# MeteoSwiss/flexpart

Hardware: AMD Instinct MI355X
Metric: particle-steps/sec (whole node) + achieved HBM GB/s, 1e8 particles (higher is better)
Workload: dtype f64

## Files before the change

__graft_entry__.py:

```python
from __future__ import annotations

import os
import subprocess
import sys

ROOT = os.path.dirname(os.path.abspath(__file__))
CSRC = os.path.join(ROOT, "flexpart_amd", "csrc")
HIPCC = os.environ.get("HIPCC", "/opt/rocm/bin/hipcc")


def _stale(out, srcs):
    if not os.path.exists(out):
        return True
    t = os.path.getmtime(out)
    return any(os.path.getmtime(s) > t for s in srcs)


UNITS = [(rb, part) for rb in (8, 4) for part in (0, 1, 2)]
HIPFLAGS = ["--offload-arch=gfx950", "-O3", "-std=c++17", "-fPIC",
            "-mllvm", "-disable-machine-licm"]


def build_library(force=False, only=None, extra_flags=(), tag=None):
    if extra_flags and not tag:
        raise ValueError("a build with extra flags needs a tag (it must not replace the product library)")
    srcs = [os.path.join(CSRC, f) for f in ("fpx_engine.hip", "fpx_device.hpp", "fpx_rng_host.hpp", "fpx_verttransform.hpp",
                                            "fpx_calcpar.hpp", "fpx_getvdep.hpp", "fpx_calcpv.hpp", "fpx_convect.hpp", "fpx_tu.hpp")]
    srcs.append(os.path.join(ROOT, "include", "flexpart_amd.h"))
    out = os.path.join(CSRC, f"libflexpart_amd_{tag}.so" if tag else "libflexpart_amd.so")
    objdir = os.path.join(CSRC, "build", tag) if tag else os.path.join(CSRC, "build")
    os.makedirs(objdir, exist_ok=True)
    flagrec = " ".join(HIPFLAGS + list(extra_flags))

    def stamp_ok(obj):
        try:
            return open(obj + ".flags").read() == flagrec
        except OSError:
            return False

    todo = []
    for rb, part in UNITS:
        name = f"r{rb}p{part}"
        obj = os.path.join(objdir, f"fpx_{name}.o")
        if only is not None and name not in only and os.path.exists(obj) and stamp_ok(obj):
            continue
        if only is not None and name in only or force or _stale(obj, srcs) or not stamp_ok(obj):
            todo.append((name, obj, rb, part))
    procs = []
    for name, obj, rb, part in todo:
        cmd = [HIPCC] + HIPFLAGS + list(extra_flags) + [f"-DFPX_TU_REAL={rb}", f"-DFPX_TU_PART={part}", "-c", os.path.join(CSRC, "fpx_engine.hip"), "-o", obj]
# ... 66 lines not shown
```

flexpart_amd/csrc/fpx_device.hpp:

```cpp
#pragma once
#include "fpx_tu.hpp"
#include <hip/hip_runtime.h>
#include <stdint.h>

namespace fpx {
FPX_TU_OPEN

#define K(x) ((R)(x))
#define FPX_DEV __device__ __forceinline__
#define FPX_HD __host__ __device__ __forceinline__

constexpr int kMaxSpec = 5;
constexpr int kMaxNests = 4;
constexpr int kDead = -999999999;

FPX_HD float m_exp(float x) { return expf(x); }
FPX_HD double m_exp(double x) { return exp(x); }
FPX_HD float m_log(float x) { return logf(x); }
FPX_HD double m_log(double x) { return log(x); }
FPX_HD float m_sqrt(float x) { return sqrtf(x); }
FPX_HD double m_sqrt(double x) { return sqrt(x); }
FPX_HD float m_fma(float a, float b, float c) { return fmaf(a, b, c); }
FPX_HD double m_fma(double a, double b, double c) { return fma(a, b, c); }
FPX_HD float m_sin(float x) { return sinf(x); }
FPX_HD double m_sin(double x) { return sin(x); }
FPX_HD float m_cos(float x) { return cosf(x); }
// ... 142 lines not shown
  const double f = fma(m, ic, -1.0);
  double p = m_fma_k(f, -1.0 / 6.0, 0.2);
  p = m_fma_k(f, p, -0.25);
  p = m_fma_k(f, p, 1.0 / 3.0);
  p = fma(f, p, -0.5);
  p = fma(f, p, 1.0);
  return fma((double)e, 6.93147180559945309417e-01, lc) + f * p;
}
FPX_DEV double m_log_abs(double x) { return m_log_abs(x, &kLogTab[0][0]); }
template <typename TP>
FPX_DEV double m_exp_tab(double x, TP tab ) {
  const double k = rint(x * 46.16624130844683);
  double r = fma(k, -0.02166084938653512, x);
  r = fma(k, -5.9631716539705866e-12, r);
  const int ki = (int)k;
  const double t = tab[ki & 31];
  double p = m_fma_k(r, 1.3888888888888888889e-03, 8.3333333333333333333e-03);
  p = m_fma_k(r, p, 4.1666666666666666667e-02);
  p = m_fma_k(r, p, 1.6666666666666666667e-01);
  p = fma(r, p, 0.5);
  p = fma(r, p, 1.0);
  return ldexp(fma(t, r * p, t), ki >> 5);
}
FPX_DEV double m_rcbrt(double x) {
  double r = (double)__builtin_amdgcn_exp2f(__log2f((float)x) * (-1.0f / 3.0f));
  const double third = 1.0 / 3.0;
#pragma unroll
  for (int it = 0; it < 2; it++) {
    const double e = fma(-(x * (r * r)), r, 1.0);
    r = fma(r * third, e, r);
  }
  return r;
}
FPX_DEV float m_expp(float x) { return __expf(x); }
FPX_DEV double m_expp(double x) {
  const double k = rint(x * 1.4426950408889634074);
  double r = fma(k, -6.93147180369123816490e-01, x);
  r = fma(k, -1.90821492927058770002e-10, r);
  const double r2 = r * r;
  double pe = fma(r2, 1.1470745597729724714e-11, 2.0876756987868098979e-09);
  pe = fma(r2, pe, 2.7557319223985890653e-07);
  pe = fma(r2, pe, 2.4801587301587301587e-05);
  pe = fma(r2, pe, 1.3888888888888888889e-03);
  pe = fma(r2, pe, 4.1666666666666666667e-02);
  pe = fma(r2, pe, 0.5);
  double po = fma(r2, 1.6059043836821614599e-10, 2.5052108385441718775e-08);
// ... 13 lines not shown
template <typename T>
FPX_DEV T m_erf_e(T x, T E) {
  const T ax = m_abs(x);
  const T xc = m_min(ax, (T)6.5);
  const T t = (xc - (T)3.0) * m_rcp(xc + (T)3.0);
  T p = (T)kErfC[0];
#pragma unroll
  for (int i = 1; i < 18; i++) p = p * t + (T)kErfC[i];
  const T r = (T)1.0 - E * p;
  return m_sign(r, x);
}
template <typename T>
FPX_DEV void m_erf_e2(T xa, T Ea, T xb, T Eb, T &ra, T &rb) {
  typedef const double __attribute__((address_space(4))) *const_ptr;
  const_ptr c = (const_ptr)kErfC;
  asm volatile("" : "+s"(c));
  const T aa = m_abs(xa), ab = m_abs(xb);
  const T ca = m_min(aa, (T)6.5), cb = m_min(ab, (T)6.5);
  const T ta = (ca - (T)3.0) * m_rcp(ca + (T)3.0), tb = (cb - (T)3.0) * m_rcp(cb + (T)3.0);
  T pa = (T)c[0], pb = (T)c[0];
#pragma unroll
  for (int i = 1; i < 18; i++) { const T k = (T)c[i]; pa = pa * ta + k; pb = pb * tb + k; }
  const T qa = (T)1.0 - Ea * pa, qb = (T)1.0 - Eb * pb;
  ra = m_sign(qa, xa);
  rb = m_sign(qb, xb);
}
FPX_DEV float m_powr(float x, float y) { return x > 0.0f ? expf(y * logf(x)) : powf(x, y); }
FPX_DEV double m_powr(double x, double y) { return m_expp(y * m_logp(x)); }
FPX_DEV float m_coslat(float x) { return cosf(x); }
FPX_DEV double m_coslat(double x) {
  if (!(fabs(x) < 1.7)) return cos(x);
  const double z = x * x;
  double p = -1.0 / 403291461126605635584000000.0;
  p = fma(p, z, 1.0 / 620448401733239439360000.0);
  p = fma(p, z, -1.0 / 1124000727777607680000.0);
  p = fma(p, z, 1.0 / 2432902008176640000.0);
  p = fma(p, z, -1.0 / 6402373705728000.0);
  p = fma(p, z, 1.0 / 20922789888000.0);
  p = fma(p, z, -1.0 / 87178291200.0);
  p = fma(p, z, 1.0 / 479001600.0);
  p = fma(p, z, -1.0 / 3628800.0);
  p = fma(p, z, 1.0 / 40320.0);
  p = fma(p, z, -1.0 / 720.0);
  p = fma(p, z, 1.0 / 24.0);
  p = fma(p, z, -0.5);
  return fma(p, z, 1.0);
// ... 592 lines not shown
  S_UST, S_WST2, S_OL, S_TRANS,
  S_IAUX, S_SIGU, S_ITLU,
  S_RHOAUX,
  S_NPASS,
  S_COUNT_LEAN,
  S_TDEP = S_COUNT_LEAN,
  S_SETCELL,
  S_SET_NUM, S_SET_DQ6, S_SET_V0,
  S_COUNT_AERO64,
  S_RT_TAG = S_COUNT_AERO64, S_RT_RHO1, S_RT_TT1, S_RT_RHO2, S_RT_TT2,
  S_COUNT
};
template <typename R> constexpr int stash_slots(bool lean, bool susp = true) { return lean ? (susp ? (int)S_COUNT_LEAN : (int)S_NPASS) : (sizeof(R) == 8 ? (int)S_COUNT_AERO64 : (int)S_COUNT); }
constexpr int kStashStride = 256;
template <typename R>
struct Stash {
  typedef __attribute__((address_space(3))) volatile R *lds_ptr;
  lds_ptr p;
  lds_tab_ptr tab;
  FPX_DEV double logabs(double x) const { return m_log_abs(x, tab); }
  FPX_DEV double expt(double x) const { return m_exp_tab(x, tab + kLdsExpTabAt); }
  FPX_DEV float logabs(float x) const { return m_logp(x); }
  FPX_DEV float expt(float x) const { return m_expp(x); }
  FPX_DEV R get(int k) const { return p[k * kStashStride]; }
  FPX_DEV void put(int k, R v) const { p[k * kStashStride] = v; }
  FPX_DEV void add(int k, R v) const { p[k * kStashStride] = p[k * kStashStride] + v; }
};

template <typename R>
FPX_DEV R inv_pack_itlu(const StepInv<R> &I) { return m_flip(I.itlu, (I.flags & INV_DEEP) ? 0x80000000u : 0u); }
FPX_DEV bool m_signbit(double x) { return __double2hiint(x) < 0; }
FPX_DEV bool m_signbit(float x) { return (int)__float_as_uint(x) < 0; }
template <typename R>
struct StashInv {
  const Stash<R> &S;
  FPX_DEV int regime() const { const R iaux = S.get(S_IAUX); return iaux > K(0.) ? 0 : iaux < K(0.) ? 1 : 2; }
  FPX_DEV bool deep() const { return m_signbit(S.get(S_ITLU)); }
  FPX_DEV R get_iaux() const { return S.get(S_IAUX); }
  FPX_DEV R get_sigu() const { return S.get(S_SIGU); }
  FPX_DEV R get_itlu() const { return m_abs(S.get(S_ITLU)); }
  FPX_DEV R get_wst2() const { return S.get(S_WST2); }
};

template <typename R>
struct HsInv {
  R ih, iaux;
  int regime;
};

template <typename R, typename ST>
// ... 29 lines not shown
    T.isigw = m_rcp(T.sigw);
    T.tlw = K(0.1) * T.h * T.isigw * m_pow08(T.zeta);
  }
  T.tlu = m_max(K(10.), T.tlu);
  T.tlv = m_max(K(10.), T.tlv);
  T.tlw = m_max(K(30.), T.tlw);
  if (sizeof(R) == 8) { if (__builtin_expect(T.dsigwdz == K(0.), 0)) { asm volatile("" ::: "memory"); T.dsigwdz = K(1.e-10); } }
  else if (T.dsigwdz == K(0.)) T.dsigwdz = K(1.e-10);
}

#define FPX_PI_PAR K(3.14159265)

template <typename R>
FPX_DEV R cuberoot(R x) { return m_sign(m_pow(m_abs(x), K(0.333333333)), x); }

template <typename R>
FPX_DEV R cbl_transition(R h, R ol) {
  R transition = K(1.);
  if (-h / ol < K(15)) transition = m_sin(((-h / ol + K(10.)) / K(10.)) * FPX_PI_PAR) / K(2.) + K(0.5);
  return transition;
}

template <typename R, typename ST>
FPX_DEV void cbl(const ST &S, int ldirect, R wp, R zp, R wt , R ih , R rhoaux , R sigmaw, R irw , R dsigmawdz, R tlw,
                 R &ath, R &bth, int &flagrein) {
  const R usurad2 = K(0.7071067812), usurad2p = K(0.3989422804), C0 = K(3), costluar4 = K(0.66667), eps = K(0.000001);
  const unsigned int tdir = ldirect < 0 ? 0x80000000u : 0u;
  const R z = zp * ih;
  const R w2 = sigmaw * sigmaw;
  const R rtl = m_rsqrt(tlw);
  const R alfa = (K(2.) / C0) * w2 * (rtl * rtl);
  const R wold = m_flip(wp, tdir);
  const R omz = K(1.) - z;
  const R omz05 = m_sqrtp(omz), omz15 = omz * omz05;
  const R w3 = (K(1.2) * z * omz15 + eps) * wt;
  const R dw3 = (K(1.2) * (omz15 - z * K(1.5) * omz05)) * (wt * ih);
  const R irw2 = irw * irw, irw3 = irw2 * irw;
  const R skew = w3 * irw3;
  const R dskew = irw3 * dw3 - K(3.) * skew * dsigmawdz * irw;
  R fluarw = K(0.), dfluarw = K(0.), xluarw = K(0.), dxluarw = K(0.);
  if (skew != K(0)) {
    R croot, icroot2;
    m_cuberoot_parts(m_abs(skew), croot, icroot2);
    fluarw = costluar4 * m_sign(croot, skew);
    dfluarw = costluar4 * (K(1.) / K(3.)) * icroot2 * dskew;
  }
  const R fluarw2 = fluarw * fluarw;
  const R a1 = K(1.) + fluarw2, a3 = K(3.) + fluarw2;
  const R ffd = K(2.) * fluarw * dfluarw;
  R a105, ia105;
  m_sqrt_rsqrt(a1, a105, ia105);
  if (skew != K(0)) {
    const R a115 = a1 * a105;
    const R ix = m_rcp(a3 * fluarw);
// ... 5 lines not shown
  m_sqrt_rsqrt(r4, r405, ir405);
  const R aluarw = K(0.5) * (K(1.) - xluarw * ir405);
  const R bluarw = K(1.) - aluarw;
  const R ir4 = ir405 * ir405;
  const R daluarw = K(-2.) * dxluarw * (ir405 * ir4);
  const R dbluarw = -daluarw;
  const R rs = r405 * ia105, rs3 = rs * (rs * rs);
  const R qa05 = bluarw * rs, qb05 = aluarw * rs;
  const R sigmawa = sigmaw * qa05, sigmawb = sigmaw * qb05;
  const R iv = irw * (a105 * r405);
  const R isa = iv * aluarw, isb = iv * bluarw;
  const R da1 = daluarw * a1, abf = ir4 * ffd, hs3 = K(0.5) * sigmaw * rs3;
  const R dsigmawa = dsigmawdz * qa05 - hs3 * bluarw * (da1 + abf);
  const R dsigmawb = dsigmawdz * qb05 + hs3 * aluarw * (da1 - abf);
  const R wa = fluarw * sigmawa, wb = fluarw * sigmawb;
  const R dwa = dfluarw * sigmawa + fluarw * dsigmawa;
  const R dwb = dfluarw * sigmawb + fluarw * dsigmawb;
  const R deltawa = wold - wa, deltawb = wold + wb;
  const R wold2 = wold * wold;
  const R isa2 = isa * isa, isb2 = isb * isb;
  const R da = deltawa * isa, db = deltawb * isb;
  if (m_abs(da) > K(6.) && m_abs(db) > K(6.)) flagrein = 1;
  const R da2 = da * da, db2 = db * db;
  const R ea = S.expt(-(K(0.5) * da2)), eb = S.expt(-(K(0.5) * db2));
  const R pa = (usurad2p * isa) * ea;
  const R pb = (usurad2p * isb) * eb;
  const R aperfa = da * usurad2;
  const R aperfb = db * usurad2;
  const R rx = rhoaux;
  const R apa = aluarw * pa, bpb = bluarw * pb;
  const R ptot = apa + bpb;
  const R Ta = aluarw * (dwa + wa * rx) + wa * daluarw;
  const R Tb = bluarw * (dwb + wb * rx) + wb * dbluarw;
  const R wdf = wold * dfluarw;
  const R Ua = sigmawa * (aluarw * (dsigmawa * (wold2 * isa2 + K(1.)) + wdf) + sigmawa * (daluarw + rx * aluarw));
  const R Ub = sigmawb * (bluarw * (dsigmawb * (wold2 * isb2 + K(1.)) - wdf) + sigmawb * (dbluarw + rx * bluarw));
  const R cu = usurad2 * usurad2 - K(0.5);
  R erfa, erfb;
  m_erf_e2(aperfa, ea - ea * (da2 * cu), aperfb, eb - eb * (db2 * cu), erfa, erfb);
  const R Phi = K(0.5) * (Tb * erfb - Ta * erfa) + Ua * pa + Ub * pb;
  const R Q = m_flip((da * isa) * apa + (db * isb) * bpb, tdir);
  ath = m_rcp(ptot) * (-(C0 / K(2.)) * alfa * Q + Phi);
  bth = (sigmaw * K(1.4142135623730951)) * rtl;
}

template <typename R>
FPX_DEV void cbl_pdf(R zp, R wst, R h, R sigmaw, R ol, R &aluarw, R &sigmawa, R &sigmawb, R &wa, R &wb) {
  const R costluar4 = K(0.66667), eps = K(0.000001);
  R z = zp / h;
  R transition = cbl_transition(h, ol);
  R w2 = sigmaw * sigmaw;
  const R omz = K(1.) - z;
  R w3 = ((K(1.2) * z * (omz * m_sqrt(omz)) + eps) * (wst * wst * wst)) * transition;
  R radw2 = m_sqrt(w2);
  R skew = w3 / (w2 * radw2);
  R skew2 = skew * skew;
  R fluarw = costluar4 * m_powr(skew, K(0.333333333333333));
  R fluarw2 = fluarw * fluarw;
  const R a1 = K(1.) + fluarw2, a3 = K(3.) + fluarw2;
  R rluarw = (a1 * a1 * a1) * skew2 / ((a3 * a3) * fluarw2);
  R xluarw = m_sqrt(rluarw);
  aluarw = K(0.5) * (K(1.) - xluarw / m_sqrt(K(4.) + rluarw));
  R bluarw = K(1.) - aluarw;
  sigmawa = radw2 * m_sqrt(bluarw / (aluarw * a1));
  sigmawb = radw2 * m_sqrt(aluarw / (bluarw * a1));
// ... 851 lines not shown
      const R y2 = k < 3 ? (h2 ? a3[lev][1][k] : a3[lev][0][k]) : (h2 ? a2[lev][1][k - 3] : a2[lev][0][k - 3]);
      y[k] = (y1 * W.dt2 + y2 * W.dt1) * W.dtt;
    }
#pragma unroll
    for (int k = 0; k < 5; k++) lv[lev][k] = y[k];
  }
}

constexpr int kRecStride = 16, kRecWst = 9;
template <typename R>
struct RecCold {
  const R *v0;
  unsigned int slot;
  FPX_DEV R wst() const {
    unsigned int s = slot;
    asm volatile("" : "+v"(s));
    return v0[(size_t)s * kRecStride + kRecWst];
  }
};

template <int T>
FPX_DEV bool sw(int runtime) { return T < 0 ? runtime != 0 : T != 0; }

template <typename R, bool DRYDEP, bool SETTLE, int TSW, int CBLF, typename RNG>
FPX_DEV int pbl_pass(const View<R> &V, const R *hgt, const RNG &G, const TimeW<R> &W, int itime, double xt, double yt,
                     R &zt, R &wp, int &ldt, short &icbt, LoopCtx<R> &A, const Stash<R> &S,
                     int &indz_last, Stats *st, const RecCold<R> &RC) {
  const R eps = V.eps;
  const R eps2 = K(1.e-9);
  const R href = K(15.);
  const R h = A.h;
  const Fld<R> F = fld_of(V, A.ngrid);
  int nrand = A.nrand;
  const bool turbswitch = sw<TSW>(V.turbswitch);
  const bool cblflag = sw<CBLF>(V.cblflag == 1);
  const bool turboff = TSW < 0 && V.turboff != 0;
  Turb<R> T;
  T.h = h;
  T.sigw = K(0.); T.dsigw2dz = K(0.); T.dsigwdz = K(0.);

  if (V.method == 1) {
    ldt = min(ldt, abs(V.lsynctime - A.itimec + itime));
    A.itimec = A.itimec + ldt * V.ldirect;
  } else {
    ldt = abs(V.lsynctime);
    A.itimec = itime + V.lsynctime;
  }
  const R dt = (R)ldt;
  T.zeta = zt / h;
// ... 48 lines not shown
    R au, bu, av, bv;
    factors(dt * itlu, au, bu);
    if (regime_h == 1) { av = au; bv = bu; }
    else factors(dt * itlv, av, bv);
    R up = S.get(S_UP), vp = S.get(S_VP);
    up = au * up + g1 * T.sigu * bu;
    vp = av * vp + g2 * T.sigv * bv;
    if (turboff) { up = K(0.); vp = K(0.); }
    S.put(S_UP, up); S.put(S_VP, vp);
    S.add(S_DAW, up * dt);
    S.add(S_DCW, vp * dt);
  }
  nrand = nrand + 2;

  if (nrand + V.ifine > V.maxrand) nrand = 1;
  const R dtf = dt * V.fine;
  const R dtftlw = dtf * m_rcp(T.tlw);
  const bool cbl_on = cblflag && SI.deep();
  const R sqrt_dtf = m_sqrtp(dtf);
  const HsInv<R> HI{ih, SI.get_iaux(), SI.regime()};

  FPX_LANES(st, 0);
  unsigned int flip = icbt < 0 ? 0x80000000u : 0u;
  for (int i = 1; i <= V.ifine; i++) {
    R delz;
    FPX_LANES(st, 1);
    if (turbswitch) {
      if (dtftlw < K(.5)) {
        if (cblflag) {
          if (cbl_on) {
            FPX_LANES(st, 2);
            int flagrein = 0;
            nrand = nrand + 1;
            R old_wp_buf = wp, ath, bth;
            cbl(S, V.ldirect, wp, zt, S.get(S_TRANS), HI.ih, S.get(S_RHOAUX), T.sigw, T.isigw, T.dsigwdz, T.tlw, ath, bth, flagrein);
            wp = m_flip(wp + ath * dtf + bth * G.at(nrand) * sqrt_dtf, flip);
            delz = wp * dtf;
            if (__builtin_expect(flagrein == 1, 0)) {
              const R wst = RC.wst();
              re_initialize_particle(V.ldirect, G, zt, wst, h, T.sigw, old_wp_buf, nrand, S.get(S_OL));
              wp = old_wp_buf;
              delz = wp * dtf;
              atomicAdd(&st->nan_count, 1ull);
            }
          } else {
            FPX_LANES(st, 3);
            nrand = nrand + 1;
            R ath = -wp * m_rcp(T.tlw) + T.sigw * T.dsigwdz + wp * wp * T.isigw * T.dsigwdz + T.sigw * T.sigw * S.get(S_RHOAUX);
            R bth = T.sigw * G.at(nrand) * m_sqrtp(K(2.) * dtftlw);
            wp = m_flip(wp + ath * dtf + bth, flip);
            delz = wp * dtf;
            if (__builtin_expect(!isfinite(wp), 0)) {
              nrand = nrand + 1;
              wp = T.sigw * G.at(nrand);
              delz = wp * dtf;
              atomicAdd(&st->nan_count2, 1ull);
            }
          }
// ... 649 lines not shown
```

flexpart_amd/csrc/fpx_engine.hip:

```cpp
#include <hip/hip_runtime.h>
#include <cstddef>
#include <cstring>
#include <rccl/rccl.h>
#include <rocprim/device/device_radix_sort.hpp>
#include <rocprim/device/device_scan.hpp>
#include <rocprim/device/device_select.hpp>
#include <rocprim/iterator/counting_iterator.hpp>
#include <algorithm>
#include <cmath>
#include <cstdio>
#include <cstring>
#include <string>
#include <vector>

#include "../../include/flexpart_amd.h"
#include "fpx_tu.hpp"
#include "fpx_device.hpp"
#include "fpx_verttransform.hpp"
#include "fpx_calcpar.hpp"
#include "fpx_getvdep.hpp"
#include "fpx_calcpv.hpp"
#include "fpx_convect.hpp"
#include "fpx_rng_host.hpp"

// ... 1083 lines not shown
                                                     unsigned int *__restrict__ next_list) {
#if !defined(FPX_VIEW_BY_VALUE) && !defined(FPX_LOOP_ONLY_VIEW)
  struct KArgs { View<R> V; Parts<R> P; PblRec<R> Q; };
  const KArgs &ka = *(const KArgs *)(const void *)__builtin_amdgcn_kernarg_segment_ptr();
  const View<R> &V = ka.V; const Parts<R> &P = ka.P; const PblRec<R> &Q = ka.Q;
  (void)V_arg; (void)P_arg; (void)Q_arg;
#else
  FPX_VIEW_FROM_KERNARG(V, V_arg);
  const Parts<R> &P = P_arg; const PblRec<R> &Q = Q_arg;
#endif
  const unsigned int *mine = blk;
  unsigned int *next_cnt = blk + kCtrStride;
  const unsigned int nlist_all = mine[0] + mine[1] + mine[2] + mine[3];
  if ((unsigned long long)blockIdx.x * kBlock >= (unsigned long long)nlist_all) return;
  const bool can_suspend = SUSP && (drain_lanes > 0 || cap_passes > 0);
  extern __shared__ __align__(16) unsigned char fpx_loop_smem[];
  static_assert(kStashStride == kBlock, "stash layout is one column per thread of the block");
  R *stash_mem = reinterpret_cast<R *>(fpx_loop_smem);
  R *hgt = stash_mem + stash_slots<R>(LEAN, SUSP) * kStashStride;
  for (int k = threadIdx.x; k < V.nz; k += blockDim.x) hgt[k] = V.height[k];
  __shared__ double lds_tab[sizeof(R) == 8 ? kLdsTabDoubles : 1];
  if (sizeof(R) == 8)
    for (int k = threadIdx.x; k < kLdsTabDoubles; k += blockDim.x) lds_tab[k] = k < kLdsExpTabAt ? kLogTab[k >> 1][k & 1] : kExpTab[k - kLdsExpTabAt];
  __syncthreads();
  const Stash<R> S{(typename Stash<R>::lds_ptr)(stash_mem + threadIdx.x), (lds_tab_ptr)lds_tab};
  const int lane = threadIdx.x & 63;
  const TimeW<R> W = time_weights(V, itime);
  const R cap_r = cap_passes > 0 ? (R)cap_passes : (R)1e30;

  unsigned int cur = 0, end = 0;
  unsigned int cbase = 0;
  unsigned int ahead = 0;
  bool out_of_chunks = false;
  int wcls = 0;
  unsigned int cls_out = 0u;
  unsigned int cls_n = mine[0], cls_seg = mine[8];
#define FPX_IN_VGPR(x) asm volatile("" : "+v"(x))
  if (SUSP) { FPX_IN_VGPR(cbase); FPX_IN_VGPR(cls_out); FPX_IN_VGPR(cls_n); FPX_IN_VGPR(cls_seg); }
#ifdef FPX_LANE_STATS
  const unsigned long long t_s = wall_clock64();
  unsigned long long t_x = 0;
#endif

  bool have = false;
  unsigned int s = 0, pid = 0;
  double xt = 0, yt = 0;
  R zt = 0, wp = 0;
  int ldt = 0;
// ... 180 lines not shown

__global__ void k_math_probe(int fn, const double *__restrict__ x, double *__restrict__ y, long long n) {
  const long long i = (long long)blockIdx.x * blockDim.x + threadIdx.x;
  if (i >= n) return;
  const double v = x[i];
  double r = 0.0, c, ic2;
  switch (fn) {
    case 0: r = m_expp(v); break;
    case 1: r = m_logp(v); break;
    case 2: r = m_sqrtp(v); break;
    case 3: r = m_rcp(v); break;
    case 4: r = m_rsqrt(v); break;
    case 5: m_cuberoot_parts(v, c, ic2); r = c; break;
    case 7: r = m_erf_e(v, m_expp(-(v * v))); break;
    case 8: r = m_pow08(v); break;
    case 9: r = m_exp_tab(v, &kExpTab[0]); break;
    case 10: r = m_log_abs(v); break;
    case 11: r = m_rcbrt(v); break;
    default: m_cuberoot_parts(v, c, ic2); r = ic2; break;
  }
  y[i] = r;
}

__global__ void __launch_bounds__(kBlock) k_hanna_probe(int which, const double *__restrict__ in, double *__restrict__ out, long long n) {
  __shared__ double slots[(S_ITLU + 1) * kStashStride];
  __shared__ double lds_tab[kLdsTabDoubles];
  for (int k = threadIdx.x; k < kLdsTabDoubles; k += blockDim.x) lds_tab[k] = k < kLdsExpTabAt ? kLogTab[k >> 1][k & 1] : kExpTab[k - kLdsExpTabAt];
  __syncthreads();
  const long long i = (long long)blockIdx.x * blockDim.x + threadIdx.x;
  if (i >= n) return;
  const double h = in[5 * i], ol = in[5 * i + 1], ust = in[5 * i + 2], wst = in[5 * i + 3], z = in[5 * i + 4];
  double *o = out + 10 * i;
  Turb<double> T;
  T.ol = ol; T.h = h; T.zeta = z / h; T.sigw = 0.; T.dsigwdz = 0.;
  if (which == 0) {
    const Stash<double> S{(Stash<double>::lds_ptr)(slots + threadIdx.x), (lds_tab_ptr)lds_tab};
    const StepInv<double> I = step_invariants(h, ol, ust, wst, PlainMath());
    S.put(S_UST, I.ust); S.put(S_OL, ol); S.put(S_WST2, wst * wst);
    S.put(S_IAUX, I.iaux); S.put(S_SIGU, I.sigu); S.put(S_ITLU, inv_pack_itlu(I));
    const StashInv<double> SI{S};
    T.ust = S.get(S_UST);
    double itlu, itlv;
    hanna(T, z, SI, S, itlu, itlv);
    o[0] = T.sigu; o[1] = T.sigv; o[2] = T.sigw; o[3] = T.dsigwdz; o[4] = itlu; o[5] = itlv; o[6] = T.tlw;
    o[7] = T.ust; o[8] = (double)SI.regime(); o[9] = SI.deep() ? 1. : 0.;
  } else {
// ... 4018 lines not shown
  return FPX_OK;
}
int fpx_count_particles(fpx_handle h, int64_t local[2], int64_t total[2], int32_t allreduce) { FPX_GUARD(h); return h->impl->count_particles(local, total, allreduce); }
int fpx_set_release_heights(fpx_handle h, int32_t numpoint, const void *zpoint1, const void *zpoint2) { FPX_GUARD(h); return h->impl->set_release_heights(numpoint, zpoint1, zpoint2); }
int fpx_set_option(fpx_handle h, const char *name, const char *value) { FPX_GUARD(h); if (!name || !value) return fpx::fail(FPX_ERR_ARG, "fpx_set_option: null argument"); return h->impl->set_option(name, value); }
int fpx_get_info(fpx_handle h, const char *name, int64_t *value) { FPX_GUARD(h); if (!name || !value) return fpx::fail(FPX_ERR_ARG, "fpx_get_info: null argument"); return h->impl->get_info(name, value); }
int fpx_lane_stats(fpx_handle h, uint64_t *out, int32_t n, int32_t reset) { FPX_GUARD(h); if (!out || n < 0) return fpx::fail(FPX_ERR_ARG, "fpx_lane_stats: bad argument"); return h->impl->lane_stats(out, n, reset); }
int fpx_comm_init(fpx_handle h, const void *id, int32_t nbytes, int32_t nranks, int32_t rank) { FPX_GUARD(h); return h->impl->comm_init(id, nbytes, nranks, rank); }
int fpx_comm_init_host(fpx_handle h, int32_t nranks, int32_t rank, fpx_allreduce_fn fn, void *user) { FPX_GUARD(h); return h->impl->comm_init_host(nranks, rank, fn, user); }
int fpx_nests_init(fpx_handle h, const fpx_nests *n) { FPX_GUARD(h); return h->impl->nests_init(n); }
int fpx_upload_nest_fields(fpx_handle h, int32_t nest, int32_t slot, const fpx_fields *f) { FPX_GUARD(h); return h->impl->upload_nest_fields(nest, slot, f); }
int fpx_wet_init(fpx_handle h, const fpx_wet_config *w) { FPX_GUARD(h); return h->impl->wet_init(w); }
int fpx_upload_wet_fields(fpx_handle h, int32_t slot, const fpx_wet_fields *f) { FPX_GUARD(h); return h->impl->upload_wet_fields(slot, f); }
int fpx_wetdepo(fpx_handle h, int32_t itime, int32_t ltsample, int32_t loutnext) { FPX_GUARD(h); return h->impl->wetdepo(itime, ltsample, loutnext); }
int fpx_get_wetgrid(fpx_handle h, void *wetgridunc, int32_t allreduce) { FPX_GUARD(h); return h->impl->get_wetgrid(wetgridunc, allreduce); }
void *fpx_stream(fpx_handle h) { return (h && h->impl) ? h->impl->stream_ptr() : nullptr; }
int fpx_upload_wet_nest_fields(fpx_handle h, int32_t nest, int32_t slot, const fpx_wet_fields *f, int32_t readclouds_nest) { FPX_GUARD(h); return h->impl->upload_wet_nest_fields(nest, slot, f, readclouds_nest); }
int fpx_outgrid_nest_init(fpx_handle h, const fpx_outgrid_nest *g) { FPX_GUARD(h); return h->impl->outgrid_nest_init(g); }
int fpx_get_grids_nest(fpx_handle h, void *griduncn, void *drygriduncn, void *wetgriduncn, int32_t allreduce, int32_t clear) { FPX_GUARD(h); return h->impl->get_grids_nest(griduncn, drygriduncn, wetgriduncn, allreduce, clear); }
int fpx_receptors_init(fpx_handle h, int32_t numreceptor, const void *xreceptor, const void *yreceptor, const void *receptorarea) { FPX_GUARD(h); return h->impl->receptors_init(numreceptor, xreceptor, yreceptor, receptorarea); }
int fpx_get_receptors(fpx_handle h, void *creceptor, int32_t ld, int32_t allreduce, int32_t clear) { FPX_GUARD(h); return h->impl->get_receptors(creceptor, ld, allreduce, clear); }

int fpx_math_probe(int32_t fn, const double *x, double *y, int64_t n) {
  if (fn < 0 || fn > 11 || !x || !y || n < 0) return FPX_ERR_ARG;
  if (n == 0) return FPX_OK;
  double *dx = nullptr, *dy = nullptr;
  if (hipMalloc(&dx, n * sizeof(double)) != hipSuccess) return FPX_ERR_NOMEM;
  if (hipMalloc(&dy, n * sizeof(double)) != hipSuccess) { (void)hipFree(dx); return FPX_ERR_NOMEM; }
  hipError_t e = hipMemcpy(dx, x, n * sizeof(double), hipMemcpyHostToDevice);
  if (e == hipSuccess) {
    fpx::k_math_probe<<<(unsigned)((n + fpx::kBlock - 1) / fpx::kBlock), fpx::kBlock>>>(fn, dx, dy, n);
    e = hipGetLastError();
  }
  if (e == hipSuccess) e = hipMemcpy(y, dy, n * sizeof(double), hipMemcpyDeviceToHost);
  (void)hipFree(dx); (void)hipFree(dy);
  return e == hipSuccess ? FPX_OK : FPX_ERR_DEVICE;
}

int fpx_hanna_probe(const double *in, double *out, int64_t n) {
  if (!in || !out || n < 0) return FPX_ERR_ARG;
  if (n == 0) return FPX_OK;
  double *dx = nullptr, *dy = nullptr;
  if (hipMalloc(&dx, 5 * n * sizeof(double)) != hipSuccess) return FPX_ERR_NOMEM;
  if (hipMalloc(&dy, 10 * n * sizeof(double)) != hipSuccess) { (void)hipFree(dx); return FPX_ERR_NOMEM; }
  hipError_t e = hipMemcpy(dx, in, 5 * n * sizeof(double), hipMemcpyHostToDevice);
  for (int which = 0; which < 2 && e == hipSuccess; which++) {
    fpx::k_hanna_probe<<<(unsigned)((n + fpx::kBlock - 1) / fpx::kBlock), fpx::kBlock>>>(which, dx, dy, n);
    e = hipGetLastError();
    if (e == hipSuccess) e = hipMemcpy(out + 10 * n * which, dy, 10 * n * sizeof(double), hipMemcpyDeviceToHost);
  }
  (void)hipFree(dx); (void)hipFree(dy);
  return e == hipSuccess ? FPX_OK : FPX_ERR_DEVICE;
}

// ... 35 lines not shown
```

Before: 384.3 million.

## Replace erf series with LDS-tabulated erfcx polynomials and fold constants in cbl

In the lean f64 path, the change swaps the 18-term erf series in the convective boundary layer (cbl) routine for a piecewise degree-10 polynomial fit of the scaled erfcx. The table sits in LDS and is indexed by interval. It also adds an exp variant that takes the squared argument directly and folds the 1/sqrt(2pi) and C0/2 constants into fewer multiplies. The zeta product is hoisted out of the ifine loop. This cuts FP64 ALU work per CBL step, but adds LDS footprint and table loads, which could lower occupancy or add LDS latency. Accuracy now depends on the fitted table.

```diff
diff --git a/__graft_entry__.py b/__graft_entry__.py
--- a/__graft_entry__.py
+++ b/__graft_entry__.py
@@ -25,7 +25,8 @@
     if extra_flags and not tag:
         raise ValueError("a build with extra flags needs a tag (it must not replace the product library)")
     srcs = [os.path.join(CSRC, f) for f in ("fpx_engine.hip", "fpx_device.hpp", "fpx_rng_host.hpp", "fpx_verttransform.hpp",
-                                            "fpx_calcpar.hpp", "fpx_getvdep.hpp", "fpx_calcpv.hpp", "fpx_convect.hpp", "fpx_tu.hpp")]
+                                            "fpx_calcpar.hpp", "fpx_getvdep.hpp", "fpx_calcpv.hpp", "fpx_convect.hpp", "fpx_tu.hpp",
+                                            "fpx_erfcx_tab.hpp")]
     srcs.append(os.path.join(ROOT, "include", "flexpart_amd.h"))
     out = os.path.join(CSRC, f"libflexpart_amd_{tag}.so" if tag else "libflexpart_amd.so")
     objdir = os.path.join(CSRC, "build", tag) if tag else os.path.join(CSRC, "build")
diff --git a/flexpart_amd/csrc/fpx_device.hpp b/flexpart_amd/csrc/fpx_device.hpp
--- a/flexpart_amd/csrc/fpx_device.hpp
+++ b/flexpart_amd/csrc/fpx_device.hpp
@@ -2,6 +2,7 @@
 #include "fpx_tu.hpp"
 #include <hip/hip_runtime.h>
 #include <stdint.h>
+#include "fpx_erfcx_tab.hpp"
 
 namespace fpx {
 FPX_TU_OPEN
@@ -190,6 +191,20 @@
   p = fma(r, p, 1.0);
   return ldexp(fma(t, r * p, t), ki >> 5);
 }
+template <typename TP>
+FPX_DEV double m_exp_tab_nh(double u, TP tab ) {
+  const double k = rint(u * -23.083120654223414);
+  double r = fma(k, 0.04332169877307024, u);
+  r = fma(k, 1.1926343307941173e-11, r);
+  const int ki = (int)k;
+  const double t = tab[ki & 31];
+  double p = m_fma_k(r, 1.3888888888888888889e-03 / 64.0, -8.3333333333333333333e-03 / 32.0);
+  p = m_fma_k(r, p, 4.1666666666666666667e-02 / 16.0);
+  p = m_fma_k(r, p, -1.6666666666666666667e-01 / 8.0);
+  p = fma(r, p, 0.125);
+  p = fma(r, p, -0.5);
+  return ldexp(fma(t, r * p, t), ki >> 5);
+}
 FPX_DEV double m_rcbrt(double x) {
   double r = (double)__builtin_amdgcn_exp2f(__log2f((float)x) * (-1.0f / 3.0f));
   const double third = 1.0 / 3.0;
@@ -249,6 +264,34 @@
 #pragma unroll
   for (int i = 1; i < 18; i++) { const T k = (T)c[i]; pa = pa * ta + k; pb = pb * tb + k; }
   const T qa = (T)1.0 - Ea * pa, qb = (T)1.0 - Eb * pb;
+  ra = m_sign(qa, xa);
+  rb = m_sign(qb, xb);
+}
+typedef __attribute__((address_space(3))) const double *lds_erft_ptr;
+template <typename TP>
+FPX_DEV double m_erfcx_tab(double c , TP tab ) {
+  static_assert(kErfcxRow >= kErfcxDegree + 2, "a row is its centre and degree + 1 coefficients");
+  const unsigned int i = min((unsigned int)(int)(c * kErfcxPerUnit), (unsigned int)(kErfcxIntervals - 1));
+  TP row = tab + i * kErfcxRow;
+  const double centre = row[0];
+  double p = row[1], w = row[2];
+  const double d = c - centre;
+#pragma unroll
+  for (int k = 2; k < kErfcxDegree + 2; k++) {
+    const double v = w;
+    if (k + 1 < kErfcxDegree + 2) {
+      asm volatile("" : "+v"(row), "+v"(p));
+      w = row[k + 1];
+    }
+    p = fma(p, d, v);
+  }
+  return p;
+}
+template <typename TP>
+FPX_DEV void m_erf_tab2(double xa, double Ea, double xb, double Eb, TP tab, double &ra, double &rb) {
+  const double pa = m_erfcx_tab(m_min(m_abs(xa), kErfcxMax), tab);
+  const double pb = m_erfcx_tab(m_min(m_abs(xb), kErfcxMax), tab);
+  const double qa = 1.0 - Ea * pa, qb = 1.0 - Eb * pb;
   ra = m_sign(qa, xa);
   rb = m_sign(qb, xb);
 }
@@ -887,10 +930,26 @@
   FPX_DEV double expt(double x) const { return m_exp_tab(x, tab + kLdsExpTabAt); }
   FPX_DEV float logabs(float x) const { return m_logp(x); }
   FPX_DEV float expt(float x) const { return m_expp(x); }
+  FPX_DEV double exp_nh(double u) const { return m_exp_tab_nh(u, tab + kLdsExpTabAt); }
+  FPX_DEV float exp_nh(float u) const { return m_expp(-(0.5f * u)); }
+  template <typename T> FPX_DEV void erf_pair(T xa, T Ea, T xb, T Eb, T &ra, T &rb) const { m_erf_e2(xa, Ea, xb, Eb, ra, rb); }
   FPX_DEV R get(int k) const { return p[k * kStashStride]; }
   FPX_DEV void put(int k, R v) const { p[k * kStashStride] = v; }
   FPX_DEV void add(int k, R v) const { p[k * kStashStride] = p[k * kStashStride] + v; }
 };
+
+struct StashErfTab : Stash<double> {
+  lds_erft_ptr erft;
+  FPX_DEV void erf_pair(double xa, double Ea, double xb, double Eb, double &ra, double &rb) const { m_erf_tab2(xa, Ea, xb, Eb, erft, ra, rb); }
+};
+template <typename R, bool ERFTAB> struct StashFor { typedef Stash<R> type; };
+template <> struct StashFor<double, true> { typedef StashErfTab type; };
+template <typename R, bool ERFTAB>
+FPX_DEV typename StashFor<R, ERFTAB>::type make_stash(typename Stash<R>::lds_ptr p, lds_tab_ptr tab, lds_erft_ptr erft) {
+  if constexpr (ERFTAB) return StashErfTab{{p, tab}, erft};
+  else return Stash<R>{p, tab};
+}
+template <typename R> constexpr bool stash_has_erf_tab(bool lean) { return lean && sizeof(R) == 8; }
 
 template <typename R>
 FPX_DEV R inv_pack_itlu(const StepInv<R> &I) { return m_flip(I.itlu, (I.flags & INV_DEEP) ? 0x80000000u : 0u); }
@@ -966,14 +1025,13 @@
 }
 
 template <typename R, typename ST>
-FPX_DEV void cbl(const ST &S, int ldirect, R wp, R zp, R wt , R ih , R rhoaux , R sigmaw, R irw , R dsigmawdz, R tlw,
+FPX_DEV void cbl(const ST &S, int ldirect, R wp, R z , R wt , R ih , R rhoaux , R sigmaw, R irw , R dsigmawdz, R tlw,
                  R &ath, R &bth, int &flagrein) {
-  const R usurad2 = K(0.7071067812), usurad2p = K(0.3989422804), C0 = K(3), costluar4 = K(0.66667), eps = K(0.000001);
+  const R usurad2 = K(0.7071067812), usurad2p = K(0.3989422804), costluar4 = K(0.66667), eps = K(0.000001);
   const unsigned int tdir = ldirect < 0 ? 0x80000000u : 0u;
-  const R z = zp * ih;
   const R w2 = sigmaw * sigmaw;
   const R rtl = m_rsqrt(tlw);
-  const R alfa = (K(2.) / C0) * w2 * (rtl * rtl);
+  const R w2tl = w2 * (rtl * rtl);
   const R wold = m_flip(wp, tdir);
   const R omz = K(1.) - z;
   const R omz05 = m_sqrtp(omz), omz15 = omz * omz05;
@@ -1025,9 +1083,9 @@
   const R da = deltawa * isa, db = deltawb * isb;
   if (m_abs(da) > K(6.) && m_abs(db) > K(6.)) flagrein = 1;
   const R da2 = da * da, db2 = db * db;
-  const R ea = S.expt(-(K(0.5) * da2)), eb = S.expt(-(K(0.5) * db2));
-  const R pa = (usurad2p * isa) * ea;
-  const R pb = (usurad2p * isb) * eb;
+  const R ea = S.exp_nh(da2), eb = S.exp_nh(db2);
+  const R pa = isa * ea;
+  const R pb = isb * eb;
   const R aperfa = da * usurad2;
   const R aperfb = db * usurad2;
   const R rx = rhoaux;
@@ -1040,10 +1098,10 @@
   const R Ub = sigmawb * (bluarw * (dsigmawb * (wold2 * isb2 + K(1.)) - wdf) + sigmawb * (dbluarw + rx * bluarw));
   const R cu = usurad2 * usurad2 - K(0.5);
   R erfa, erfb;
-  m_erf_e2(aperfa, ea - ea * (da2 * cu), aperfb, eb - eb * (db2 * cu), erfa, erfb);
-  const R Phi = K(0.5) * (Tb * erfb - Ta * erfa) + Ua * pa + Ub * pb;
+  S.erf_pair(aperfa, ea - ea * (da2 * cu), aperfb, eb - eb * (db2 * cu), erfa, erfb);
+  const R Phi = (K(0.5) / usurad2p) * (Tb * erfb - Ta * erfa) + Ua * pa + Ub * pb;
   const R Q = m_flip((da * isa) * apa + (db * isb) * bpb, tdir);
-  ath = m_rcp(ptot) * (-(C0 / K(2.)) * alfa * Q + Phi);
+  ath = m_rcp(ptot) * (Phi - w2tl * Q);
   bth = (sigmaw * K(1.4142135623730951)) * rtl;
 }
 
@@ -1941,9 +1999,9 @@
 template <int T>
 FPX_DEV bool sw(int runtime) { return T < 0 ? runtime != 0 : T != 0; }
 
-template <typename R, bool DRYDEP, bool SETTLE, int TSW, int CBLF, typename RNG>
+template <typename R, bool DRYDEP, bool SETTLE, int TSW, int CBLF, typename RNG, typename ST >
 FPX_DEV int pbl_pass(const View<R> &V, const R *hgt, const RNG &G, const TimeW<R> &W, int itime, double xt, double yt,
-                     R &zt, R &wp, int &ldt, short &icbt, LoopCtx<R> &A, const Stash<R> &S,
+                     R &zt, R &wp, int &ldt, short &icbt, LoopCtx<R> &A, const ST &S,
                      int &indz_last, Stats *st, const RecCold<R> &RC) {
   const R eps = V.eps;
   const R eps2 = K(1.e-9);
@@ -2038,6 +2096,8 @@
 
   FPX_LANES(st, 0);
   unsigned int flip = icbt < 0 ? 0x80000000u : 0u;
+  constexpr bool zeta_is_product = CBLF > 0;
+  if (zeta_is_product) T.zeta = zt * HI.ih;
   for (int i = 1; i <= V.ifine; i++) {
     R delz;
     FPX_LANES(st, 1);
@@ -2049,7 +2109,7 @@
             int flagrein = 0;
             nrand = nrand + 1;
             R old_wp_buf = wp, ath, bth;
-            cbl(S, V.ldirect, wp, zt, S.get(S_TRANS), HI.ih, S.get(S_RHOAUX), T.sigw, T.isigw, T.dsigwdz, T.tlw, ath, bth, flagrein);
+            cbl(S, V.ldirect, wp, zeta_is_product ? T.zeta : zt * HI.ih, S.get(S_TRANS), HI.ih, S.get(S_RHOAUX), T.sigw, T.isigw, T.dsigwdz, T.tlw, ath, bth, flagrein);
             wp = m_flip(wp + ath * dtf + bth * G.at(nrand) * sqrt_dtf, flip);
             delz = wp * dtf;
             if (__builtin_expect(flagrein == 1, 0)) {
diff --git a/flexpart_amd/csrc/fpx_engine.hip b/flexpart_amd/csrc/fpx_engine.hip
--- a/flexpart_amd/csrc/fpx_engine.hip
+++ b/flexpart_amd/csrc/fpx_engine.hip
@@ -1129,8 +1129,13 @@
   __shared__ double lds_tab[sizeof(R) == 8 ? kLdsTabDoubles : 1];
   if (sizeof(R) == 8)
     for (int k = threadIdx.x; k < kLdsTabDoubles; k += blockDim.x) lds_tab[k] = k < kLdsExpTabAt ? kLogTab[k >> 1][k & 1] : kExpTab[k - kLdsExpTabAt];
+  constexpr bool ERFTAB = stash_has_erf_tab<R>(LEAN);
+  __shared__ __align__(16) double lds_erft[ERFTAB ? kErfcxIntervals * kErfcxRow : 2];
+  if (ERFTAB)
+    for (int k = threadIdx.x; k < kErfcxIntervals * kErfcxRow; k += blockDim.x) lds_erft[k] = kErfcxTab[k];
   __syncthreads();
-  const Stash<R> S{(typename Stash<R>::lds_ptr)(stash_mem + threadIdx.x), (lds_tab_ptr)lds_tab};
+  typedef typename StashFor<R, ERFTAB>::type stash_t;
+  const stash_t S = make_stash<R, ERFTAB>((typename Stash<R>::lds_ptr)(stash_mem + threadIdx.x), (lds_tab_ptr)lds_tab, (lds_erft_ptr)lds_erft);
   const int lane = threadIdx.x & 63;
   const TimeW<R> W = time_weights(V, itime);
   const R cap_r = cap_passes > 0 ? (R)cap_passes : (R)1e30;
@@ -1357,6 +1362,24 @@
   y[i] = r;
 }
 
+__global__ void __launch_bounds__(kBlock) k_erf_probe(int fn, const double *__restrict__ in, double *__restrict__ y, long long n) {
+  __shared__ __align__(16) double lds_erft[kErfcxIntervals * kErfcxRow];
+  for (int k = threadIdx.x; k < kErfcxIntervals * kErfcxRow; k += blockDim.x) lds_erft[k] = kErfcxTab[k];
+  __syncthreads();
+  const long long i = (long long)blockIdx.x * blockDim.x + threadIdx.x;
+  if (i >= n) return;
+  const double v = in[i];
+  if (fn == 14) { y[i] = m_exp_tab_nh(v, &kExpTab[0]); return; }
+  const double E = in[n + i];
+  const long long j = i + 1 < n ? i + 1 : 0;
+  const double v2 = in[j], E2 = in[n + j];
+  double a, b, c, d;
+  if (fn == 12) { m_erf_e2(v, E, v2, E2, a, b); m_erf_e2(v2, E2, v, E, c, d); }
+  else { m_erf_tab2(v, E, v2, E2, (lds_erft_ptr)lds_erft, a, b); m_erf_tab2(v2, E2, v, E, (lds_erft_ptr)lds_erft, c, d); }
+  const bool same = a == d || (a != a && d != d);
+  y[i] = same ? a : __builtin_nan("");
+}
+
 __global__ void __launch_bounds__(kBlock) k_hanna_probe(int which, const double *__restrict__ in, double *__restrict__ out, long long n) {
   __shared__ double slots[(S_ITLU + 1) * kStashStride];
   __shared__ double lds_tab[kLdsTabDoubles];
@@ -5421,14 +5444,16 @@
 int fpx_get_receptors(fpx_handle h, void *creceptor, int32_t ld, int32_t allreduce, int32_t clear) { FPX_GUARD(h); return h->impl->get_receptors(creceptor, ld, allreduce, clear); }
 
 int fpx_math_probe(int32_t fn, const double *x, double *y, int64_t n) {
-  if (fn < 0 || fn > 11 || !x || !y || n < 0) return FPX_ERR_ARG;
+  if (fn < 0 || fn > 14 || !x || !y || n < 0) return FPX_ERR_ARG;
   if (n == 0) return FPX_OK;
+  const int64_t nin = (fn == 12 || fn == 13) ? 2 * n : n;
   double *dx = nullptr, *dy = nullptr;
-  if (hipMalloc(&dx, n * sizeof(double)) != hipSuccess) return FPX_ERR_NOMEM;
+  if (hipMalloc(&dx, nin * sizeof(double)) != hipSuccess) return FPX_ERR_NOMEM;
   if (hipMalloc(&dy, n * sizeof(double)) != hipSuccess) { (void)hipFree(dx); return FPX_ERR_NOMEM; }
-  hipError_t e = hipMemcpy(dx, x, n * sizeof(double), hipMemcpyHostToDevice);
+  hipError_t e = hipMemcpy(dx, x, nin * sizeof(double), hipMemcpyHostToDevice);
   if (e == hipSuccess) {
-    fpx::k_math_probe<<<(unsigned)((n + fpx::kBlock - 1) / fpx::kBlock), fpx::kBlock>>>(fn, dx, dy, n);
+    if (fn >= 12) fpx::k_erf_probe<<<(unsigned)((n + fpx::kBlock - 1) / fpx::kBlock), fpx::kBlock>>>(fn, dx, dy, n);
+    else fpx::k_math_probe<<<(unsigned)((n + fpx::kBlock - 1) / fpx::kBlock), fpx::kBlock>>>(fn, dx, dy, n);
     e = hipGetLastError();
   }
   if (e == hipSuccess) e = hipMemcpy(y, dy, n * sizeof(double), hipMemcpyDeviceToHost);
diff --git a/flexpart_amd/csrc/fpx_erfcx_tab.hpp b/flexpart_amd/csrc/fpx_erfcx_tab.hpp
--- /dev/null
+++ b/flexpart_amd/csrc/fpx_erfcx_tab.hpp
@@ -0,0 +1,33 @@
+#pragma once
+namespace fpx {
+constexpr int kErfcxIntervals = 26, kErfcxDegree = 10, kErfcxRow = 12;
+constexpr double kErfcxPerUnit = 4.0, kErfcxMax = 6.5;
+static __device__ const double kErfcxTab[kErfcxIntervals * kErfcxRow] = {
+  0x1.0000000000000p-3, 0x1.3855acaf76de7p-8, -0x1.705f0259d8f6ap-7, 0x1.9a9e16d8ab91cp-6, -0x1.b503f3e0bd91fp-5, 0x1.b5f0a1120dfe6p-4, -0x1.99c4e1c600512p-3, 0x1.6210c62495355p-2, -0x1.163c18bf5a6c1p-1, 0x1.84d8493cb1c0ep-1, -0x1.d1f52e46ef8d5p-1, 0x1.bf16ef058facfp-1,
+  0x1.8000000000000p-2, 0x1.a4fc216357e0fp-10, -0x1.066b6c106ff9fp-8, 0x1.366178999afcbp-7, -0x1.5f758a6ff1efep-6, 0x1.784920378791cp-5, -0x1.7a16153d24dbcp-4, 0x1.611afb944367dp-3, -0x1.2e82dbf82432dp-2, 0x1.d28c0e1177cfep-2, -0x1.3a5c679d7bb91p-1, 0x1.5f28ade3ca4acp-1,
+  0x1.4000000000000p-1, 0x1.2c1238408959bp-11, -0x1.8b48ee8729b41p-10, 0x1.efce943a006d1p-9, -0x1.2a7e22bbf5142p-7, 0x1.552fe75cce8ffp-6, -0x1.6fce5e74788e5p-5, 0x1.72d46a9b2e7d4p-4, -0x1.59c35c06e077ep-3, 0x1.2577420fcd08ap-2, -0x1.babd0e4f1a272p-2, 0x1.1d16b5809eaf6p-1,
+  0x1.c000000000000p-1, 0x1.c2f23aabebb55p-13, -0x1.39ab6559fb41cp-11, 0x1.a0ee5f44c3b93p-10, -0x1.0ab2ac7ccdb7fp-8, 0x1.452649151d6a2p-7, -0x1.779dd301d1310p-6, 0x1.9831c2c844c5ep-5, -0x1.9d5868ddfa8fap-4, 0x1.80ef8f454cf91p-3, -0x1.4369f60195eeap-2, 0x1.db747ee409ac5p-2,
+  0x1.2000000000000p+0, 0x1.640e780ceea15p-14, -0x1.055ff1ee8d6a1p-12, 0x1.6fd8d831bfdd4p-11, -0x1.f38b2b04878abp-10, 0x1.446c5193b941dp-8, -0x1.910a5dc281c24p-7, 0x1.d4e711a2d791dp-6, -0x1.01343a2c8bdb5p-4, 0x1.05e72521ca1bbp-3, -0x1.e78b356770fc5p-3, 0x1.9531e09b149b5p-2,
+  0x1.6000000000000p+0, 0x1.2681f63d17129p-15, -0x1.c7f450ab7929bp-14, 0x1.535ebe4e7b38fp-12, -0x1.e8ad6b8e491c4p-11, 0x1.51aba01e88a08p-9, -0x1.bdf24c0411cbep-8, 0x1.17eba60d2efbdp-6, -0x1.4bcdb9d90349bp-5, 0x1.701342cbcea7dp-4, -0x1.797a639d812a1p-3, 0x1.5f88f52f3c76bp-2,
+  0x1.a000000000000p+0, 0x1.fcdda4901ad15p-17, -0x1.9f01ec6586418p-15, 0x1.465e54bb6234bp-13, -0x1.f1b36d327890cp-12, 0x1.6d609f850717ep-10, -0x1.014eae3ef31d9p-8, 0x1.5a142948a758ep-7, -0x1.ba018e6423ff8p-6, 0x1.0a15ac2adab36p-4, -0x1.2b11e6959934dp-3, 0x1.3583f6644327bp-2,
+  0x1.e000000000000p+0, 0x1.c9e257a15716dp-18, -0x1.890a4fdb7d217p-16, 0x1.4631625d248bdp-14, -0x1.070db39a9ad32p-12, 0x1.99b60e586134bp-11, -0x1.33237c526a465p-9, 0x1.b99589d40d37fp-8, -0x1.2ef92f6f0ebbbp-6, 0x1.8a6efeed233adp-5, -0x1.e36580c7f734cp-4, 0x1.13e5743b60480p-2,
+  0x1.1000000000000p+1, 0x1.abfb46f696656p-19, -0x1.8241dc2b70fc5p-17, 0x1.51e032ccba60fp-15, -0x1.1fc841cc67a9dp-13, 0x1.dab55d81adb5ap-12, -0x1.7a18193718d14p-10, 0x1.21decee0ed27bp-8, -0x1.aa2443aac5be2p-7, 0x1.2adaf7aaf55e2p-5, -0x1.8d6f73d5aa122p-4, 0x1.f0fd28fdc20abp-3,
+  0x1.3000000000000p+1, 0x1.9e7ecd21e9267p-20, -0x1.88e1729fee449p-18, 0x1.69c2fbd6d62c8p-16, -0x1.44f89f7079813p-14, 0x1.1b649ba2ed531p-12, -0x1.deb45ead0961ep-11, 0x1.8680d287487f7p-9, -0x1.32a8abc8da822p-7, 0x1.cdc880a056a24p-6, -0x1.4baeac94dc8b2p-4, 0x1.c3987d04d0b98p-3,
+  0x1.5000000000000p+1, 0x1.9ef7cf3c74cb4p-21, -0x1.9c9e589650a95p-19, 0x1.8f68f0e9335d5p-17, -0x1.79da7d6a11fb2p-15, 0x1.5bd1dd6a5de72p-13, -0x1.36e99414da5e2p-11, 0x1.0d40a2ab36431p-9, -0x1.c28dd3c4d5c80p-8, 0x1.6afd3ba3fa642p-6, -0x1.18737afe106cep-4, 0x1.9d7738e1f4db7p-3,
+  0x1.7000000000000p+1, 0x1.ac8041bb5c766p-22, -0x1.be73495a13dc0p-20, 0x1.c5b44a4bdc35dp-18, -0x1.c35c1fefa637cp-16, 0x1.b5d78b34b3b83p-14, -0x1.9d6f222eef8f0p-12, 0x1.7b404aa4de7ccp-10, -0x1.512f92fca680fp-8, 0x1.21c23afa33c47p-6, -0x1.dfc0205709b2cp-5, 0x1.7d0a5e9dd5710p-3,
+  0x1.9000000000000p+1, 0x1.c772834f868e6p-23, -0x1.f0a240dc74febp-21, 0x1.08947ab39a48fp-18, -0x1.146336ae1ff87p-16, 0x1.1a12c4a6b177ap-14, -0x1.18d4654b8d95cp-12, 0x1.104973fea30e3p-10, -0x1.009a927223847p-8, 0x1.d503e1d20090ep-7, -0x1.9e8803e177224p-5, 0x1.612a8125451bdp-3,
+  0x1.b000000000000p+1, 0x1.f15401ba86e09p-24, -0x1.1b73623a02634p-21, 0x1.3c3b5084ad94cp-19, -0x1.5a6113c021becp-17, 0x1.7350e3a365bb7p-15, -0x1.85118471a6425p-13, 0x1.8de5f26a7e3e2p-11, -0x1.8c84c13afb6e4p-9, 0x1.804cc15714188p-7, -0x1.696d353f008b5p-5, 0x1.48f8f10299b71p-3,
+  0x1.d000000000000p+1, 0x1.16764438b5331p-24, -0x1.4b6db9531387bp-22, 0x1.82a8fb8d40c0fp-20, -0x1.bb73860fa2784p-18, 0x1.f28b1c3a08a29p-16, -0x1.1267afc6eed73p-13, 0x1.276b01ef6f847p-11, -0x1.36992d37bbe86p-9, 0x1.3e68313870541p-7, -0x1.3dacc8d85f6c4p-5, 0x1.33cb19179d7f6p-3,
+  0x1.f000000000000p+1, 0x1.3f441d09ff9fdp-25, -0x1.8c4fa4eaddfb1p-23, 0x1.e2df6fca58431p-21, -0x1.2186f3f3cf921p-18, 0x1.54d6c39de72c6p-16, -0x1.898597a085badp-14, 0x1.bd21af8e75d13p-12, -0x1.ecb581c2b7dcbp-10, 0x1.0a7a05d3387a8p-7, -0x1.193eb7b9bf564p-5, 0x1.211c625924e34p-3,
+  0x1.0800000000000p+2, 0x1.763539309636ap-26, -0x1.e3e8fb80db145p-24, 0x1.338069b220666p-21, -0x1.810d9ffd655efp-19, 0x1.d9f64545be2a0p-17, -0x1.1e807be5afe4ep-14, 0x1.53e39641d549ep-12, -0x1.8b46c64f91d87p-10, 0x1.c21d6f4a4921ap-8, -0x1.f53cfd5c11186p-6, 0x1.10845e1dcb19ap-3,
+  0x1.1800000000000p+2, 0x1.bfc002ac02782p-27, -0x1.2d433e70db40ep-24, 0x1.8ee2bb47b3bcbp-22, -0x1.0471968f03da8p-19, 0x1.4eb8a60c7f801p-17, -0x1.a712d1a27ee85p-15, 0x1.06bf9a3516c25p-12, -0x1.406f090aa3f7ap-10, 0x1.7f51652a46399p-8, -0x1.c14b6f7f3c2f0p-6, 0x1.01afcc22e71b8p-3,
+  0x1.2800000000000p+2, 0x1.111a57b62b15fp-27, -0x1.7e051807f7e71p-25, 0x1.072c10d831defp-22, -0x1.65f1095d1b507p-20, 0x1.dfa9cd10d24c7p-18, -0x1.3c74896398118p-15, 0x1.9adeaa13913fap-13, -0x1.0641d50f05bd8p-10, 0x1.48ea08fa97bd8p-8, -0x1.94e4c65b27fd6p-6, 0x1.e8b725e90fb8dp-4,
+  0x1.3800000000000p+2, 0x1.5340b90464dc9p-28, -0x1.ecc6565dd0871p-26, 0x1.60d9afdcdd02cp-23, -0x1.f33ee444e2285p-21, 0x1.5c5596d439771p-18, -0x1.df2332f5533a2p-16, 0x1.44a17930a9818p-13, -0x1.b1138bae63673p-11, 0x1.1c3200b14f2f0p-8, -0x1.6ea9db64452a6p-6, 0x1.d0a2236d493eap-4,
+  0x1.4800000000000p+2, 0x1.aca98d9ff5099p-29, -0x1.42f320b742e87p-26, 0x1.e032910daf740p-24, -0x1.60fcfd4617be5p-21, 0x1.00254409fdcbfp-18, -0x1.6ecb6c32d0edbp-16, 0x1.02fdcfb106fdfp-13, -0x1.687d168ebc109p-11, 0x1.ee3ffedd01da2p-9, -0x1.4d86dc544600bp-6, 0x1.bac6ca42e1bfbp-4,
+  0x1.5800000000000p+2, 0x1.132faa17f9f93p-29, -0x1.adb587b92c0d5p-27, 0x1.4b592a4f78c27p-24, -0x1.f99c7d3d7c8bfp-22, 0x1.7d2054ac1015bp-19, -0x1.1bb8488eb4410p-16, 0x1.a0faa96f4a819p-14, -0x1.2e52cf81e3f2dp-11, 0x1.b04ef16d7ef9bp-9, -0x1.30a0ebefa7ff4p-6, 0x1.a6dab49575b6dp-4,
+  0x1.6800000000000p+2, 0x1.66add1e17d53fp-30, -0x1.21f109dbff0b8p-27, 0x1.cf4daef6e18d9p-25, -0x1.6e7de6cb1ca48p-22, 0x1.1ea5688f78b29p-19, -0x1.bb2e61502d9c4p-17, 0x1.527c1e396f01fp-14, -0x1.fe9e2a1afd58fp-12, 0x1.7c2ef77e9114dp-9, -0x1.1748bb019ff2dp-6, 0x1.949fbeb63d761p-4,
+  0x1.7800000000000p+2, 0x1.da2de9e779586p-31, -0x1.8c7e7a458bebap-28, 0x1.47e8bd34a96d0p-25, -0x1.0ca905e870b03p-22, 0x1.b3956212b5957p-20, -0x1.5d44315418890p-17, 0x1.14e914d25fdcep-14, -0x1.b1ffaa6f881dep-12, 0x1.500652770df53p-9, -0x1.00f0a28e0b70dp-6, 0x1.83e1a154593d6p-4,
+  0x1.8800000000000p+2, 0x1.3da7798033906p-31, -0x1.1282215143f48p-28, 0x1.d58e759e702cfp-26, -0x1.8e1290dd6b038p-23, 0x1.4e1f24cf60430p-20, -0x1.1594dc8871220p-17, 0x1.c85edd24048d1p-15, -0x1.7318428a380b1p-12, 0x1.2a6189daf30dep-9, -0x1.da4a7e35becddp-7, 0x1.747414effdae0p-4,
+  0x1.9800000000000p+2, 0x1.aeff99cfb49e8p-32, -0x1.809aeb4c06543p-29, 0x1.53dec2430b929p-26, -0x1.29da9dda6c4ebp-23, 0x1.0298266228743p-20, -0x1.bcb667005c4bap-18, 0x1.7a9f9dad403dbp-15, -0x1.3f1651ac0ffc0p-12, 0x1.0a1ac60286bf7p-9, -0x1.b70fb7681780ep-7, 0x1.66315c5706f0bp-4,
+};
+}
```

New measurement: 391.5 million (median of 6 runs). 1.02x the previous value.
